# ZwwWayne/mmMOT

Hardware: NVIDIA H100
Metric: frame-pairs/sec at N=128 dets (higher is better)
Workload: dtype f32 (tensor-core engine: FP16 hi/lo split operands, fp32 accumulate)

## Files before the change

mmmot_b200/csrc/gemm_tma.cuh:

```cuda
#pragma once
#include <cuda.h>
#include <cuda_fp16.h>

#include "tc_common.cuh"

namespace tma {

using namespace tc;

constexpr int T_THREADS = 384;
constexpr int T_EPI_WARPS = 8, T_LOAD_WARP = 8;
constexpr int T_CONS_REGS = 232, T_LOAD_REGS = 40;
static_assert(256 * T_CONS_REGS + 128 * T_LOAD_REGS <= launch_regs(T_THREADS) * T_THREADS, "register split exceeds the CTA's pool");
constexpr int T_EPI_SCRATCH = 32 * 80;
constexpr int T_STAGES = 4;
constexpr int T_STAGE_BYTES = A_SUB + 2 * B_HALF;
constexpr size_t T_SMEM_BYTES = (size_t)T_STAGES * T_STAGE_BYTES + 1024 + 256 + T_EPI_WARPS * T_EPI_SCRATCH;
static_assert(T_SMEM_BYTES <= 227 * 1024, "gemm_tma_kernel exceeds the 227 KB of shared memory per block");
static_assert(T_STAGES * T_STAGE_BYTES >= 128 * BN * 4, "the accumulator image must fit in the ring it overlays");

enum { OUT_PLANAR = 3 };

struct TmaP {
  TcP t;
// ... 238 lines not shown
            const uint64_t b_hi = smem_desc_sw64(sb + ks * 32), b_lo = smem_desc_sw64(sb + B_HALF + ks * 32);
#pragma unroll
            for (int mb = 0; mb < 2; mb++) {
              const uint32_t a = sa + mb * 8 * SBO + ks * 2 * A_LBO;
              const uint64_t a_hi = smem_desc(a, A_LBO, SBO), a_lo = smem_desc(a + A_HALF, A_LBO, SBO);
              wgmma_n128(acc[mb], a_hi, b_hi, ((kc - kc_lo) | ks) ? 1u : 0u);
              wgmma_n128(acc[mb], a_hi, b_lo, 1u);
              wgmma_n128(acc[mb], a_lo, b_hi, 1u);
            }
          }
          wgmma_commit();
        }
        wgmma_wait<1>();
        if (kc > kc_lo) { __syncwarp(); if (lane == 0) mbar_arrive(empty_bar((it - 1) % T_STAGES)); }
      }
      wgmma_wait<0>();
      fence_acc(acc[0]);
      fence_acc(acc[1]);
      __syncwarp();
      if (lane == 0) mbar_arrive(empty_bar((it - 1) % T_STAGES));
      bar_sync(7, T_EPI_WARPS * 32);
      acc_dump(acc[0], img, BN, 0, half * 128);
      acc_dump(acc[1], img, BN, 64, half * 128);
      bar_sync(7, T_EPI_WARPS * 32);
      if (P.ksegs > 1) {
        {
          const int co = mg * 128 + q * 32 + lane;
          const bool rowok = co < p.M;
          const float bv = (rowok && p.bias) ? __ldg(p.bias + co) : 0.f;
#pragma unroll 1
          for (int cc = 0; cc < 4; cc++) {
            const int col0 = half * 128 + cc * 32;
            uint32_t v[32];
            acc_ld32(img, BN, q * 32 + lane, col0, v);
            if (!rowok) continue;
            float* sp = P.acc_scratch + ((long)nt * BN + col0) * p.M + co;
            if (seg < P.ksegs - 1) {
              if (seg == 0) {
#pragma unroll
                for (int j = 0; j < 32; j++) __stcg(sp + (long)j * p.M, __uint_as_float(v[j]) * P.t.out_scale);
              } else {
                float sv[32];
#pragma unroll
                for (int j = 0; j < 32; j++) sv[j] = __ldcg(sp + (long)j * p.M);
#pragma unroll
                for (int j = 0; j < 32; j++) __stcg(sp + (long)j * p.M, fmaf(__uint_as_float(v[j]), P.t.out_scale, sv[j]));
              }
            } else {
              float sv[32];
#pragma unroll
              for (int j = 0; j < 32; j++) sv[j] = __ldcg(sp + (long)j * p.M);
#pragma unroll
              for (int j = 0; j < 32; j++) {
                float a = fmaf(__uint_as_float(v[j]), P.t.out_scale, sv[j]) + bv;
                sv[j] = p.relu ? fmaxf(a, 0.f) : a;
              }
              emit_conv(sv, cc, col0, co, i0, y0, x0);
            }
          }
          if (P.pool && seg == P.ksegs - 1 && rowok) pool_flush(co);
        }
      } else
      {
        const int co = mg * 128 + q * 32 + lane;
        const bool rowok = co < p.M;
        const float bv = (rowok && p.bias) ? __ldg(p.bias + co) : 0.f;
        double f1 = 0.0, f2 = 0.0;
        const bool pass2 = P.segsum && !p.part && !p.Y && !p.relu;
        const bool use_seg = p.seg && (p.addend || P.segsum);
        int4 ct = make_int4(0, 0, 0, 0);
        if (use_seg) ct = __ldg(P.chunk_tab + (long)nt * 2 + half);
        const int cdesc[4] = {ct.x, ct.y, ct.z, ct.w};
        float adv[4] = {0.f, 0.f, 0.f, 0.f};
        unsigned one_det = 0;
#pragma unroll
        for (int c = 0; c < 4; c++) {
          if (cdesc[c] & 1) {
            one_det |= 1u << c;
            if (p.addend && rowok) adv[c] = __ldg(p.addend + (long)(cdesc[c] >> 1) * p.ld_add + co);
          }
        }
        float na = 0.f, nb = 0.f;
        if (P.segsum && rowok) { na = __ldg(p.sc + (long)g * p.M + co); nb = __ldg(p.sh + (long)g * p.M + co); }
#pragma unroll 1
        for (int cc = 0; cc < 4; cc++) {
          const int col0 = half * 128 + cc * 32;
          if (col0 >= len) break;
          const int da = (cc == 0 ? ct.x : cc == 1 ? ct.y : cc == 2 ? ct.z : ct.w) >> 1;
          const float adc = cc == 0 ? adv[0] : cc == 1 ? adv[1] : cc == 2 ? adv[2] : adv[3];
          const bool single = (one_det >> cc) & 1u;
          uint32_t v[32];
          acc_ld32(img, BN, q * 32 + lane, col0, v);
          if (P.t.dbg & 1) continue;
          float s1 = 0.f, s2 = 0.f, pv = 0.f;
          bool fast = col0 + 32 <= len;
          if (pass2 && fast) {
            if (single) {
              if (rowok) {
                const float bva = bv + adc;
                const float a2 = P.t.out_scale * na, b2 = fmaf(bva, na, nb);
                float r0 = 0.f, r1 = 0.f;
#pragma unroll
                for (int j = 0; j < 32; j += 2) {
                  r0 += fmaxf(fmaf(__uint_as_float(v[j]), a2, b2), 0.f);
                  r1 += fmaxf(fmaf(__uint_as_float(v[j + 1]), a2, b2), 0.f);
                }
                atomicAdd(P.segsum + (long)da * p.M + co, __float2ull_rn((r0 + r1) * 4294967296.f));
              }
              continue;
            }
          }
          float bva = bv;
          if (fast && p.addend) {
            if (single) bva += adc;
            else fast = false;
          }
          if (fast) {
            if (p.relu) epi_fast<true>(v, P.t.out_scale, bva, pv, s1, s2);
            else epi_fast<false>(v, P.t.out_scale, bva, pv, s1, s2);
          } else {
            float t = 0.f;
#pragma unroll
            for (int j = 0; j < 32; j++) {
              float x = fmaf(__uint_as_float(v[j]), P.t.out_scale, bv);
              const int col = col0 + j;
              if (p.addend && rowok && col < len)
                x += __ldg(p.addend + (long)__ldg(p.seg + c0 + col) * p.ld_add + co);
              if (p.relu) x = fmaxf(x, 0.f);
              v[j] = __float_as_uint(x);
              if (col < len) t += x;
            }
            pv = t / (float)min(32, len - col0);
#pragma unroll
            for (int j = 0; j < 32; j++)
              if (col0 + j < len) { const float d = __uint_as_float(v[j]) - pv; s1 += d; s2 = fmaf(d, d, s2); }
          }
          stat_fold(f1, f2, min(32, len - col0), pv, s1, s2);
          if (P.segsum && rowok) {
            const int nvalid = min(32, len - col0);
            int dcur = da;
            float run = 0.f;
            if (single) {
#pragma unroll
              for (int j = 0; j < 32; j++) run += fmaxf(fmaf(__uint_as_float(v[j]), na, nb), 0.f);
            } else {
#pragma unroll
              for (int j = 0; j < 32; j++) {
                if (j < nvalid) {
                  const int d = __ldg(p.seg + c0 + col0 + j);
                  if (d != dcur) {
                    atomicAdd(P.segsum + (long)dcur * p.M + co, __float2ull_rn(run * 4294967296.f));
                    run = 0.f; dcur = d;
                  }
                  run += fmaxf(fmaf(__uint_as_float(v[j]), na, nb), 0.f);
                }
              }
            }
            atomicAdd(P.segsum + (long)dcur * p.M + co, __float2ull_rn(run * 4294967296.f));
          }
          if (!p.Y || !rowok) continue;
          if (P.conv) {
            float xv[32];
#pragma unroll
            for (int j = 0; j < 32; j++) xv[j] = __uint_as_float(v[j]);
            emit_conv(xv, cc, col0, co, i0, y0, x0);
          } else {
            const int nvalid = min(32, len - col0);
            const long row0 = (long)g * p.y_gs + c0 + col0;
            if (P.t.out_mode == OUT_PLANAR && !(p.y_ms & 31)) {
              float xv[32];
#pragma unroll
              for (int j = 0; j < 32; j++) xv[j] = __uint_as_float(v[j]);
              store_rows(xv, lane < nvalid, (row0 + lane) * p.y_ms + (co - lane));
            } else if (P.t.out_mode == OUT_PLANAR) {
              __half* dst = yh + row0 * p.y_ms + co;
#pragma unroll
              for (int j = 0; j < 32; j++)
                if (j < nvalid) {
                  __half h, l;
                  split_f16(__uint_as_float(v[j]), h, l);
                  amax = fmaxf(amax, fabsf(__uint_as_float(v[j])));
                  dst[(long)j * p.y_ms] = h;
                  dst[(long)j * p.y_ms + P.plane_elems] = l;
                }
            } else {
              float* dst = p.Y + row0 * p.y_ms + co;
              if (nvalid == 32) {
#pragma unroll
                for (int j = 0; j < 32; j++) { *dst = __uint_as_float(v[j]); dst += p.y_ms; }
              } else {
#pragma unroll
                for (int j = 0; j < 32; j++)
                  if (j < nvalid) dst[(long)j * p.y_ms] = __uint_as_float(v[j]);
              }
            }
          }
        }
        if (p.part && rowok) p.part[((long)nt * 2 + half) * p.M + co] = make_double2(f1, f2);
        if (P.conv && P.pool && rowok) pool_flush(co);
      }
      fence_async_smem();
      __syncwarp();
      if (lane == 0) mbar_arrive(free_bar);
      }
    }
    mm_range_flag(P.status, amax);
  } else {
    asm volatile("setmaxnreg.dec.sync.aligned.u32 %0;" ::"n"(T_LOAD_REGS));
    if (warp == T_LOAD_WARP && lane == 0) {
      uint32_t it = 0, wcount = 0;
      for (long t = blockIdx.x; t < total_tiles; t += gridDim.x) {
        const int mg = (int)(t % mgroups);
        const int nt = (int)(t / mgroups);
        const int mt0 = mg;
        int g = 0, c0 = 0, len = BN, i0 = 0, y0 = 0, x0 = 0;
        if (P.conv) conv_origin(nt, i0, y0, x0); else tile_cols(nt, g, c0, len);
        const int row0 = (int)((long)g * p.x_gs + c0);
        for (int kc = 0; kc < KC; kc++, it++) {
          if (kc % P.kc_per_seg == 0) {
            if (wcount > 0) mbar_wait(free_bar, (wcount - 1) & 1);
            wcount++;
          }
          const int s = it % T_STAGES;
          mbar_wait(empty_bar(s), ((it / T_STAGES) & 1) ^ 1);
          const uint32_t abytes = (uint32_t)A_SUB;
          const bool skipA = P.t.dbg & 2, skipB = P.t.dbg & 4;
          mbar_expect_tx(full_bar(s), (skipA ? 0u : abytes) + (skipB ? 0u : 2u * B_HALF));
          const uint32_t sa = base + s * T_STAGE_BYTES, sb = sa + A_SUB;
          const uint8_t* src = reinterpret_cast<const uint8_t*>(P.t.Wp) + ((size_t)kc * P.t.m_tiles + mt0) * A_SUB;
          if (!skipA) bulk_g2s(sa, src, abytes, full_bar(s));
          if (skipB) continue;
          if (P.conv) {
            const int tap = kc / cchunks, cc = kc - tap * cchunks;
            const int dx = tap % 3 - 1, dy = tap / 3 - 1;
            tma_load_4d(sb, &map_hi, cc * BK, x0 + dx, y0 + dy, i0, full_bar(s));
            tma_load_4d(sb + B_HALF, &map_lo, cc * BK, x0 + dx, y0 + dy, i0, full_bar(s));
          } else {
            tma_load_2d(sb, &map_hi, kc * BK, row0, full_bar(s));
            tma_load_2d(sb + B_HALF, &map_lo, kc * BK, row0, full_bar(s));
          }
        }
      }
    }
    __syncwarp();
  }

}

typedef CUresult (*EncodeTiledFn)(CUtensorMap*, CUtensorMapDataType, cuuint32_t, void*, const cuuint64_t*,
                                  const cuuint64_t*, const cuuint32_t*, const cuuint32_t*, CUtensorMapInterleave,
                                  CUtensorMapSwizzle, CUtensorMapL2promotion, CUtensorMapFloatOOBfill);
static inline EncodeTiledFn encode_fn() {
  static EncodeTiledFn fn = nullptr;
  if (!fn) {
    void* p = nullptr;
    cudaDriverEntryPointQueryResult qr;
    if (cudaGetDriverEntryPoint("cuTensorMapEncodeTiled", &p, cudaEnableDefault, &qr) == cudaSuccess &&
        qr == cudaDriverEntryPointSuccess)
      fn = (EncodeTiledFn)p;
  }
  return fn;
}
static inline int make_map_2d(CUtensorMap* m, const void* basep, long rows, int C, long ld) {
  EncodeTiledFn fn = encode_fn();
  if (!fn) return MMMOT_E_ARG;
  cuuint64_t dims[2] = {(cuuint64_t)C, (cuuint64_t)rows};
  cuuint64_t strides[1] = {(cuuint64_t)ld * 2};
  cuuint32_t box[2] = {32, 256}, es[2] = {1, 1};
  CUresult r = fn(m, CU_TENSOR_MAP_DATA_TYPE_FLOAT16, 2, const_cast<void*>(basep), dims, strides, box, es,
                  CU_TENSOR_MAP_INTERLEAVE_NONE, CU_TENSOR_MAP_SWIZZLE_64B, CU_TENSOR_MAP_L2_PROMOTION_L2_128B,
                  CU_TENSOR_MAP_FLOAT_OOB_FILL_NONE);
  return r == CUDA_SUCCESS ? 0 : 900 + (int)r;
}
static inline int make_map_2d_f32(CUtensorMap* m, const void* basep, long rows, int C, int box_rows,
                                  CUtensorMapSwizzle swizzle) {
  EncodeTiledFn fn = encode_fn();
  if (!fn) return MMMOT_E_ARG;
  cuuint64_t dims[2] = {(cuuint64_t)C, (cuuint64_t)rows};
  cuuint64_t strides[1] = {(cuuint64_t)C * 4};
  cuuint32_t box[2] = {32, (cuuint32_t)box_rows}, es[2] = {1, 1};
  CUresult r = fn(m, CU_TENSOR_MAP_DATA_TYPE_FLOAT32, 2, const_cast<void*>(basep), dims, strides, box, es,
                  CU_TENSOR_MAP_INTERLEAVE_NONE, swizzle, CU_TENSOR_MAP_L2_PROMOTION_L2_128B,
                  CU_TENSOR_MAP_FLOAT_OOB_FILL_NONE);
  return r == CUDA_SUCCESS ? 0 : 900 + (int)r;
}
static inline int make_map_4d(CUtensorMap* m, const void* basep, int n_img, int H, int W, int C, int bx, int by,
                              int bi) {
  EncodeTiledFn fn = encode_fn();
  if (!fn) return MMMOT_E_ARG;
  cuuint64_t dims[4] = {(cuuint64_t)C, (cuuint64_t)W, (cuuint64_t)H, (cuuint64_t)n_img};
  cuuint64_t strides[3] = {(cuuint64_t)C * 2, (cuuint64_t)W * C * 2, (cuuint64_t)H * W * C * 2};
  cuuint32_t box[4] = {32, (cuuint32_t)bx, (cuuint32_t)by, (cuuint32_t)bi}, es[4] = {1, 1, 1, 1};
  CUresult r = fn(m, CU_TENSOR_MAP_DATA_TYPE_FLOAT16, 4, const_cast<void*>(basep), dims, strides, box, es,
                  CU_TENSOR_MAP_INTERLEAVE_NONE, CU_TENSOR_MAP_SWIZZLE_64B, CU_TENSOR_MAP_L2_PROMOTION_L2_128B,
                  CU_TENSOR_MAP_FLOAT_OOB_FILL_NONE);
  return r == CUDA_SUCCESS ? 0 : 900 + (int)r;
}

}

#include "gemm_tma_px.cuh"

static int gemm_tma_px_launch(tma::TmaP& P, const CUtensorMap& mh, const CUtensorMap& ml, int sms, cudaStream_t st) {
  static std::atomic<unsigned long long> attr{0};
  MM_TRY(mm_ensure_smem(tma::gemm_tma_px_kernel<false>, tma::PX_SMEM_BYTES, attr));
  const long total = P.t.g.num_tiles;
  const int grid = (int)(total < sms ? total : sms);
  tma::gemm_tma_px_kernel<false><<<grid, tma::PX_THREADS, tma::PX_SMEM_BYTES, st>>>(P, mh, ml);
  MM_LAUNCH_CHECK();
  return 0;
}

static int gemm_tma_px_launch_gen27(const float* crops, int n_img, int H, int W, const uint4* Wpx, float out_scale,
                                    const float* bias, __half* Yhi, long y_plane, int* status, cudaStream_t st) {
  if (!crops || !Wpx || !Yhi) return MMMOT_E_ARG;
  const long n_pix = (long)n_img * H * W;
  if (n_pix >= (1L << 31) || ((long)H * W) % tc::BN || (tc::BN + 2 * W + 2) * 12 > 2 * tma::PX_W_SLOT) return MMMOT_E_SHAPE;
  int sms = 0;
  MM_TRY(mm_sm_count(&sms));
  static std::atomic<unsigned long long> attr{0};
  MM_TRY(mm_ensure_smem(tma::gemm_tma_px_kernel<true>, tma::PX_SMEM_BYTES, attr));
  tma::TmaP P;
  memset(&P, 0, sizeof(P));
  GemmP g = gemm_defaults();
  g.bias = bias; g.M = 64; g.K = 32; g.relu = 1;
  g.S = (int)n_pix; g.tiles_per_group = mm_cdiv(n_pix, tc::BN); g.num_tiles = g.tiles_per_group;
  g.Y = reinterpret_cast<float*>(Yhi); g.y_ms = 64;
  P.t.g = g;
  P.t.Wp = Wpx; P.wcompact = 1;
  P.t.m_tiles = 1; P.t.k_chunks = 1;
  P.t.out_scale = out_scale;
  P.t.out_mode = tma::OUT_PLANAR;
  P.t.dbg = mm_debug_flags();
  P.plane_elems = y_plane;
  P.ksegs = 1; P.kc_per_seg = 1;
  P.status = status;
  P.gen_src = crops; P.n_img = n_img; P.H = H; P.W = W;
  alignas(64) CUtensorMap dummy;
  memset(&dummy, 0, sizeof(dummy));
  const long total = g.num_tiles;
  const int grid = (int)(total < sms ? total : sms);
  tma::gemm_tma_px_kernel<true><<<grid, tma::PX_GEN_THREADS, tma::PX_SMEM_BYTES, st>>>(P, dummy, dummy);
  MM_LAUNCH_CHECK();
  return 0;
}

static int gemm_tma_launch_mat(const GemmP& g, const uint4* Wp, float out_scale, const __half* Xhi, long x_plane,
                               long rows, int ldx, int out_mode, long y_plane, cudaStream_t st,
                               unsigned long long* segsum = nullptr, int* status = nullptr, const int4* chunk_tab = nullptr,
                               const uint4* Wpx = nullptr) {
  if (!Wp || g.num_tiles <= 0 || g.K % tc::BK) return MMMOT_E_ARG;
  int sms = 0;
  MM_TRY(mm_sm_count(&sms));
  static std::atomic<unsigned long long> attr{0};
  MM_TRY(mm_ensure_smem(tma::gemm_tma_kernel, tma::T_SMEM_BYTES, attr));
  tma::TmaP P;
  memset(&P, 0, sizeof(P));
  P.t.g = g;
  P.t.Wp = Wp;
  P.t.m_tiles = (g.M + 127) / 128;
  P.t.k_chunks = g.K / tc::BK;
  P.t.out_scale = out_scale;
  P.t.out_mode = out_mode;
  P.t.dbg = mm_debug_flags();
  P.plane_elems = y_plane;
  P.ksegs = 1; P.kc_per_seg = P.t.k_chunks;
  P.segsum = segsum;
  P.status = status;
  P.chunk_tab = chunk_tab;
  if (g.seg && (g.addend || segsum) && !chunk_tab) return MMMOT_E_ARG;
  alignas(64) CUtensorMap mh, ml;
  MM_TRY(tma::make_map_2d(&mh, Xhi, rows, g.K, ldx));
  MM_TRY(tma::make_map_2d(&ml, Xhi + x_plane, rows, g.K, ldx));
  if (out_mode == tma::OUT_PLANAR && g.M == 64 && g.y_ms == 64 && !g.part && !segsum && !g.addend && !g.tile_tab &&
      !(P.t.dbg & 64)) {
    if (Wpx) { P.t.Wp = Wpx; P.wcompact = 1; }
    return gemm_tma_px_launch(P, mh, ml, sms, st);
  }
  const long total = (long)g.num_tiles * P.t.m_tiles;
  const int grid = (int)(total < sms ? total : sms);
  tma::gemm_tma_kernel<<<grid, tma::T_THREADS, tma::T_SMEM_BYTES, st>>>(P, mh, ml);
  MM_LAUNCH_CHECK();
  return 0;
}

static inline double conv_box_waste(int n_img, int H, int W, int bx, int by, int bi) {
  return (double)mm_cdiv(W, bx) * bx / W * mm_cdiv(H, by) * by / H * mm_cdiv(n_img, bi) * bi / n_img;
}

struct ConvPlan {
  int px;
  int halo;
  int pool;
  int bx, by, bi;
  int ksegs, kc_per_seg;
  int tiles_x, tiles_y, num_tiles;
};
static inline ConvPlan conv_plan(int M, bool part, int n_img, int H, int W, int C, bool want_pool, bool use_kseg, int dbg,
                                 int seg_chunks) {
  ConvPlan c;
  memset(&c, 0, sizeof(c));
  c.bx = 1; c.by = 1; c.bi = 256;
  double best = 1e30;
  for (int cx = 256; cx >= 1; cx >>= 1)
    for (int cy = 256 / cx; cy >= 1; cy >>= 1) {
      const int ci = 256 / (cx * cy);
      const double waste = conv_box_waste(n_img, H, W, cx, cy, ci);
      if (waste < best - 1e-9) { best = waste; c.bx = cx; c.by = cy; c.bi = ci; }
    }
  const int kchunks = 9 * C / tc::BK;
  c.px = M == 64 && !part && !(dbg & 64) && !(use_kseg && seg_chunks > 0 && kchunks > seg_chunks);
  if (c.px && conv_box_waste(1, H, W, 16, 16, 1) <= best + 1e-9) { c.bx = 16; c.by = 16; c.bi = 1; }
  if (c.px) {
    c.halo = (c.bi == 1 && c.bx >= 8 && c.bx * (c.by + 2) * 64 <= tma::PX_X_PLANE && !(dbg & 256)) ? 1 : 0;
    c.pool = want_pool && c.bx >= 2 && c.bx <= 16 && c.by >= 2 && !(H & 1) && !(W & 1) && !(dbg & 512);
  } else {
    c.pool = want_pool && c.bx >= 2 && c.bx <= 32 && c.by >= 2 && !(H & 1) && !(W & 1) && !(dbg & 512);
  }
  c.ksegs = 1; c.kc_per_seg = kchunks;
  if (use_kseg && seg_chunks > 0 && kchunks > seg_chunks) {
    c.ksegs = (kchunks + seg_chunks - 1) / seg_chunks;
    c.kc_per_seg = (kchunks + c.ksegs - 1) / c.ksegs;
  }
  c.tiles_x = mm_cdiv(W, c.bx); c.tiles_y = mm_cdiv(H, c.by);
  c.num_tiles = c.tiles_x * c.tiles_y * mm_cdiv(n_img, c.bi);
  return c;
}

static int gemm_tma_launch_conv(const GemmP& g0, const uint4* Wp, float out_scale, const __half* Xhi, long x_plane,
                                int n_img, int H, int W, int C, __half* Yhi, long y_plane, cudaStream_t st,
                                float* acc_scratch = nullptr, long y_plane_pooled = 0, int* did_pool = nullptr,
                                int* status = nullptr, unsigned long long* pool_sum = nullptr, const uint4* Wpx = nullptr,
                                ConvPlan* plan = nullptr) {
  if (did_pool) *did_pool = 0;
  if (!Wp || C % tc::BK) return MMMOT_E_ARG;
  const ConvPlan c = conv_plan(g0.M, g0.part != nullptr, n_img, H, W, C, y_plane_pooled > 0 && did_pool,
                               acc_scratch != nullptr, mm_debug_flags(), mm_kseg_chunks());
  if (plan) *plan = c;
  int sms = 0;
  MM_TRY(mm_sm_count(&sms));
  static std::atomic<unsigned long long> attr{0};
  MM_TRY(mm_ensure_smem(tma::gemm_tma_kernel, tma::T_SMEM_BYTES, attr));
  tma::TmaP P;
  memset(&P, 0, sizeof(P));
  GemmP g = g0;
  g.K = 9 * C;
  P.conv = 1; P.bx = c.bx; P.by = c.by; P.bi = c.bi;
  P.halo = c.halo;
  P.pool = c.pool;
  if (c.pool) *did_pool = 1;
  if (c.pool && !c.px) P.pool_sum = pool_sum;
  P.tiles_x = c.tiles_x; P.tiles_y = c.tiles_y;
  P.n_img = n_img; P.H = H; P.W = W; P.C = C;
  g.num_tiles = c.num_tiles;
  g.tile_tab = nullptr;
  g.Y = reinterpret_cast<float*>(Yhi);
  g.y_ms = g.M;
  P.t.g = g;
  P.t.Wp = Wp;
  P.t.m_tiles = (g.M + 127) / 128;
  P.t.k_chunks = g.K / tc::BK;
  P.t.out_scale = out_scale;
  P.t.out_mode = tma::OUT_PLANAR;
  P.t.dbg = mm_debug_flags();
  P.plane_elems = P.pool ? y_plane_pooled : y_plane;
  P.status = status;
  P.ksegs = c.ksegs; P.kc_per_seg = c.kc_per_seg;
  if (c.ksegs > 1) P.acc_scratch = acc_scratch;
  alignas(64) CUtensorMap mh, ml;
  const int box_y = P.halo ? c.by + 2 : c.by;
  MM_TRY(tma::make_map_4d(&mh, Xhi, n_img, H, W, C, c.bx, box_y, c.bi));
  MM_TRY(tma::make_map_4d(&ml, Xhi + x_plane, n_img, H, W, C, c.bx, box_y, c.bi));
  if (c.px) {
    if (Wpx) { P.t.Wp = Wpx; P.wcompact = 1; }
    return gemm_tma_px_launch(P, mh, ml, sms, st);
  }
  const long total = (long)g.num_tiles * P.t.m_tiles;
  const int grid = (int)(total < sms ? total : sms);
  tma::gemm_tma_kernel<<<grid, tma::T_THREADS, tma::T_SMEM_BYTES, st>>>(P, mh, ml);
  MM_LAUNCH_CHECK();
  return 0;
}
```

mmmot_b200/csrc/gemm_tma_px.cuh:

```cuda
#pragma once

namespace tma {

constexpr int PX_W_SLOT = 8192;
constexpr int PX_W_LBO = 1024;
constexpr int PX_X_OFF = 3 * PX_W_SLOT;
constexpr int PX_X_PLANE = 24576;
constexpr int PX_STAGE = PX_X_OFF + 2 * PX_X_PLANE;
constexpr int PX_STAGES = 2;
constexpr int PX_IMG = 256 * 64 * 4;
constexpr size_t PX_SMEM_BYTES = (size_t)PX_STAGES * PX_STAGE + PX_IMG + 1024 + 256;

constexpr int PX_WC_LBO = 2048;

constexpr int PX_THREADS = 288, PX_GEN_THREADS = 640, PX_GEN_WARP0 = 12;
constexpr int PX_CONS_REGS = 144, PX_LOAD_REGS = 24, PX_PROD_REGS = 80;
static_assert(256 * PX_CONS_REGS + 128 * PX_LOAD_REGS + 256 * PX_PROD_REGS <= launch_regs(PX_GEN_THREADS) * PX_GEN_THREADS,
              "GEN27 register split exceeds the CTA's pool");

constexpr int PX_GEN_WARPS = 4;

template <bool GEN27>
static __global__ void __launch_bounds__(GEN27 ? PX_GEN_THREADS : PX_THREADS, 1)
gemm_tma_px_kernel(const TmaP P, const __grid_constant__ CUtensorMap map_hi, const __grid_constant__ CUtensorMap map_lo) {
  const GemmP& p = P.t.g;
  extern __shared__ uint8_t smem_raw[];
  __shared__ float s_bias[64];
  const uint32_t raw = smem_u32(smem_raw);
  const uint32_t base = (raw + 1023u) & ~1023u;
  uint8_t* sm = smem_raw + (base - raw);
  float* img = reinterpret_cast<float*>(sm + PX_STAGES * PX_STAGE);
  const uint32_t bar0 = base + PX_STAGES * PX_STAGE + PX_IMG;
  auto full_bar = [&](int s) { return bar0 + 8u * s; };
  auto empty_bar = [&](int s) { return bar0 + 8u * (PX_STAGES + s); };

  const int tid = threadIdx.x, warp = tid >> 5, lane = tid & 31;
  const long total_tiles = p.num_tiles;
  const int KC = P.t.k_chunks;
  const int cchunks = P.conv ? P.C / BK : KC;
  const int ntap = P.halo ? 3 : 1;
  const int nstage = P.halo ? 3 * cchunks : KC;
  const uint32_t xbytes = P.halo ? (uint32_t)(P.bx * (P.by + 2) * 64) : (uint32_t)B_HALF;

  if (tid < 64) s_bias[tid] = p.bias ? p.bias[tid] : 0.f;
  if (tid == 0) {
    for (int s = 0; s < PX_STAGES; s++) {
      mbar_init(full_bar(s), GEN27 ? 1 + PX_GEN_WARPS : 1);
      mbar_init(empty_bar(s), T_EPI_WARPS);
    }
    asm volatile("fence.mbarrier_init.release.cluster;" ::: "memory");
  }
  __syncthreads();

  auto conv_origin = [&](int nt, int& i0, int& y0, int& x0) {
    const int tx = nt % P.tiles_x;
    const int r = nt / P.tiles_x;
    const int ty = r % P.tiles_y;
    i0 = (r / P.tiles_y) * P.bi; y0 = ty * P.by; x0 = tx * P.bx;
  };

  if (warp < T_EPI_WARPS) {
    if (GEN27) asm volatile("setmaxnreg.inc.sync.aligned.u32 %0;" ::"n"(PX_CONS_REGS));
    const int q = warp & 3, cb = (warp >> 2) * 32;
    const int lbx = 31 - __clz(max(P.bx, 1)), lby = 31 - __clz(max(P.by, 1));
    __half* yh = reinterpret_cast<__half*>(p.Y);
    uint32_t racc = 0;
    uint32_t it = 0;
    const int wg = warp >> 2;
    float acc[2][32];
#pragma unroll
    for (int mb = 0; mb < 2; mb++)
#pragma unroll
      for (int i = 0; i < 32; i++) acc[mb][i] = 0.f;
    for (long t = blockIdx.x; t < total_tiles; t += gridDim.x) {
      const int nt = (int)t;
      int i0 = 0, y0 = 0, x0 = 0;
      if (P.conv) conv_origin(nt, i0, y0, x0);
      for (int si = 0; si < nstage; si++, it++) {
        const int s = it % PX_STAGES;
        mbar_wait(full_bar(s), (it / PX_STAGES) & 1);
        const uint32_t sw = base + s * PX_STAGE, sx = sw + PX_X_OFF;
        if (!(P.t.dbg & 8)) {
          wgmma_fence();
          for (int ky = 0; ky < ntap; ky++) {
            const uint32_t xo = sx + (uint32_t)(ky * P.bx * 64 + wg * (128 * 64)), wo = sw + (uint32_t)(ky * PX_W_SLOT);
#pragma unroll
            for (int ks = 0; ks < 2; ks++) {
              uint64_t w_hi, w_lo;
              if (P.wcompact) {
                w_hi = smem_desc(wo + ks * 2 * PX_WC_LBO, PX_WC_LBO, SBO);
                w_lo = smem_desc(wo + 8 * SBO + ks * 2 * PX_WC_LBO, PX_WC_LBO, SBO);
              } else {
                w_hi = smem_desc(wo + ks * 2 * PX_W_LBO, PX_W_LBO, SBO);
                w_lo = smem_desc(wo + PX_W_SLOT / 2 + ks * 2 * PX_W_LBO, PX_W_LBO, SBO);
              }
#pragma unroll
              for (int mb = 0; mb < 2; mb++) {
                const uint64_t x_hi = smem_desc_sw64(xo + mb * (64 * 64) + ks * 32);
                const uint64_t x_lo = smem_desc_sw64(xo + PX_X_PLANE + mb * (64 * 64) + ks * 32);
                wgmma_n64(acc[mb], x_hi, w_hi, (si | ky | ks) ? 1u : 0u);
                wgmma_n64(acc[mb], x_hi, w_lo, 1u);
                wgmma_n64(acc[mb], x_lo, w_hi, 1u);
              }
            }
          }
          wgmma_commit();
        }
        wgmma_wait<1>();
        if (si > 0) { __syncwarp(); if (lane == 0) mbar_arrive(empty_bar((it - 1) % PX_STAGES)); }
      }
      wgmma_wait<0>();
      fence_acc(acc[0]);
      fence_acc(acc[1]);
      __syncwarp();
      if (lane == 0) mbar_arrive(empty_bar((it - 1) % PX_STAGES));
      bar_sync(7, T_EPI_WARPS * 32);
      acc_dump(acc[0], img, 64, wg * 128, 0);
      acc_dump(acc[1], img, 64, wg * 128 + 64, 0);
      bar_sync(7, T_EPI_WARPS * 32);
#pragma unroll 1
      for (int sub = 0; sub < 2; sub++) {
        const int col = sub * 128 + q * 32 + lane;
        bool ok;
        long o;
        if (P.conv) {
          const int xx = col & (P.bx - 1), r = col >> lbx;
          const int yy = r & (P.by - 1), ii = r >> lby;
          const int img = i0 + ii, y = y0 + yy, xg = x0 + xx;
          ok = img < P.n_img && y < P.H && xg < P.W;
          o = (((long)img * P.H + y) * P.W + xg) * 64 + cb;
        } else {
          const long row = (long)nt * BN + col;
          ok = row < p.S;
          o = row * 64 + cb;
        }
        uint32_t v[32];
        acc_ld32(img, 64, sub * 128 + q * 32 + lane, cb, v);
        if (P.t.dbg & 1) continue;
        if (P.pool) {
#pragma unroll
          for (int j = 0; j < 32; j++) {
            float a = __uint_as_float(v[j]);
            a = fmaxf(a, __shfl_xor_sync(0xffffffffu, a, 1));
            a = fmaxf(a, __shfl_xor_sync(0xffffffffu, a, P.bx));
            v[j] = __float_as_uint(a);
          }
          const int xx = col & (P.bx - 1), r = col >> lbx;
          const int yy = r & (P.by - 1);
          const int y = y0 + yy, xg = x0 + xx;
          ok = ok && !(xx & 1) && !(yy & 1);
          o = (((long)(i0 + (r >> lby)) * (P.H >> 1) + (y >> 1)) * (P.W >> 1) + (xg >> 1)) * 64 + cb;
          if (!ok) continue;
        }
        uint32_t hi[16], lo[16];
#pragma unroll
        for (int j = 0; j < 32; j += 2) {
          float x0v = fmaf(__uint_as_float(v[j]), P.t.out_scale, s_bias[cb + j]);
          float x1v = fmaf(__uint_as_float(v[j + 1]), P.t.out_scale, s_bias[cb + j + 1]);
          if (p.relu) { x0v = fmaxf(x0v, 0.f); x1v = fmaxf(x1v, 0.f); }
          split_f16x2(x0v, x1v, hi[j >> 1], lo[j >> 1]);
          mm_range_track2(racc, hi[j >> 1]);
        }
        if (GEN27) {
          const uint32_t scr = base + (uint32_t)((q >> 1) * PX_STAGE + PX_X_OFF + (q & 1) * PX_X_PLANE + 16384);
          const uint32_t rowa = scr + (uint32_t)lane * 128u;
#pragma unroll
          for (int k = 0; k < 4; k++) {
            const uint32_t slot = (uint32_t)((((cb >> 3) + k) ^ (lane & 7)) << 4);
            asm volatile("st.shared.v4.b32 [%0], {%1, %2, %3, %4};" ::"r"(rowa + slot), "r"(hi[4 * k]), "r"(hi[4 * k + 1]),
                         "r"(hi[4 * k + 2]), "r"(hi[4 * k + 3]) : "memory");
            asm volatile("st.shared.v4.b32 [%0], {%1, %2, %3, %4};" ::"r"(rowa + 4096u + slot), "r"(lo[4 * k]),
                         "r"(lo[4 * k + 1]), "r"(lo[4 * k + 2]), "r"(lo[4 * k + 3]) : "memory");
          }
          asm volatile("bar.sync %0, 64;" ::"r"(3 + q) : "memory");
          const int h = warp >> 2;
          const long row0 = (long)nt * BN + sub * 128 + q * 32;
          __half* dstp = yh + (long)h * P.plane_elems + row0 * 64;
#pragma unroll
          for (int r = 0; r < 4; r++) {
            const int idx = r * 32 + lane, px = idx >> 2, c = (idx & 3) * 2;
            const uint32_t ra = scr + (uint32_t)h * 4096u + (uint32_t)px * 128u;
            uint32_t w[8];
            asm volatile("ld.shared.v4.b32 {%0, %1, %2, %3}, [%4];" : "=r"(w[0]), "=r"(w[1]), "=r"(w[2]), "=r"(w[3])
                         : "r"(ra + (uint32_t)((c ^ (px & 7)) << 4)));
            asm volatile("ld.shared.v4.b32 {%0, %1, %2, %3}, [%4];" : "=r"(w[4]), "=r"(w[5]), "=r"(w[6]), "=r"(w[7])
                         : "r"(ra + (uint32_t)(((c + 1) ^ (px & 7)) << 4)));
            if (row0 + px < p.S) st_global_256(dstp + (long)px * 64 + c * 8, w);
          }
          asm volatile("bar.sync %0, 64;" ::"r"(3 + q) : "memory");
        } else if (ok && !(P.t.dbg & 128)) {
          st_global_256(yh + o, hi);
          st_global_256(yh + o + 16, hi + 8);
          st_global_256(yh + o + P.plane_elems, lo);
          st_global_256(yh + o + P.plane_elems + 16, lo + 8);
        } else if (ok) {
          uint4* dh = reinterpret_cast<uint4*>(yh + o);
          uint4* dl = reinterpret_cast<uint4*>(yh + o + P.plane_elems);
#pragma unroll
          for (int k = 0; k < 4; k++) {
            dh[k] = make_uint4(hi[4 * k], hi[4 * k + 1], hi[4 * k + 2], hi[4 * k + 3]);
            dl[k] = make_uint4(lo[4 * k], lo[4 * k + 1], lo[4 * k + 2], lo[4 * k + 3]);
          }
        }
      }
    }
    mm_range_flag2(P.status, racc);
  } else if (GEN27 && warp >= PX_GEN_WARP0) {
    asm volatile("setmaxnreg.dec.sync.aligned.u32 %0;" ::"n"(PX_PROD_REGS));
    const int pw = warp - PX_GEN_WARP0;
    const int grp = pw >> 2;
    const int pt = (pw & 3) * 32 + lane;
    const int W = P.W, hw = P.H * P.W;
    const int span = BN + 2 * W + 2;
    float amax = 0.f;
    uint32_t it = (uint32_t)grp;
    for (long t = blockIdx.x + (long)grp * gridDim.x; t < total_tiles; t += 2L * gridDim.x, it += 2) {
      const int s = it % PX_STAGES;
      const long row0 = t * BN;
      const long img = row0 / hw;
      const int r0 = (int)(row0 - img * hw);
      const float* src = P.gen_src + img * 3 * hw;
      mbar_wait(empty_bar(s), ((it / PX_STAGES) & 1) ^ 1);
      float* stg = reinterpret_cast<float*>(sm + s * PX_STAGE + PX_W_SLOT);
      const int lin0 = r0 - W - 1;
      if (P.t.dbg & 4) {
        __syncwarp();
        if (lane == 0) mbar_arrive(full_bar(s));
        continue;
      }
#pragma unroll 1
      for (int i0 = pt; i0 < 3 * span; i0 += 8 * 128) {
        float q[8];
#pragma unroll
        for (int u = 0; u < 8; u++) {
          const int i = i0 + u * 128;
          const int ci = i / span, lin = lin0 + (i - ci * span);
          q[u] = (i < 3 * span && lin >= 0 && lin < hw) ? __ldg(src + (long)ci * hw + lin) : 0.f;
        }
#pragma unroll
        for (int u = 0; u < 8; u++)
          if (i0 + u * 128 < 3 * span) stg[i0 + u * 128] = q[u];
      }
      asm volatile("bar.sync %0, 128;" ::"r"(1 + grp) : "memory");
      const uint32_t sx = base + s * PX_STAGE + PX_X_OFF;
#pragma unroll
      for (int j = 0; j < 2; j++) {
        const int rr = j * 128 + pt;
        const int x = (r0 + rr) % W;
        const bool xl = x > 0, xr = x < W - 1;
        const float* c = stg + rr + W + 1;
        float v[28];
#pragma unroll
        for (int ci = 0; ci < 3; ci++)
#pragma unroll
          for (int ky = 0; ky < 3; ky++)
#pragma unroll
            for (int kx = 0; kx < 3; kx++) {
              float q = c[ci * span + (ky - 1) * W + (kx - 1)];
              if (kx == 0 && !xl) q = 0.f;
              if (kx == 2 && !xr) q = 0.f;
              v[ci * 9 + ky * 3 + kx] = q;
              amax = fmaxf(amax, fabsf(q));
            }
        v[27] = 0.f;
        uint32_t hi[16], lo[16];
#pragma unroll
        for (int k = 0; k < 28; k += 2) split_f16x2(v[k], v[k + 1], hi[k >> 1], lo[k >> 1]);
        hi[14] = hi[15] = lo[14] = lo[15] = 0u;
        const uint32_t rowaddr = sx + (uint32_t)rr * 64u, sw = (uint32_t)((rr >> 1) & 3);
#pragma unroll
        for (int cch = 0; cch < 4; cch++) {
          const uint32_t a = rowaddr + ((cch ^ sw) << 4);
          asm volatile("st.shared.v4.b32 [%0], {%1, %2, %3, %4};" ::"r"(a), "r"(hi[4 * cch]), "r"(hi[4 * cch + 1]),
                       "r"(hi[4 * cch + 2]), "r"(hi[4 * cch + 3]) : "memory");
          asm volatile("st.shared.v4.b32 [%0], {%1, %2, %3, %4};" ::"r"(a + PX_X_PLANE), "r"(lo[4 * cch]),
                       "r"(lo[4 * cch + 1]), "r"(lo[4 * cch + 2]), "r"(lo[4 * cch + 3]) : "memory");
        }
      }
      asm volatile("fence.proxy.async.shared::cta;" ::: "memory");
      __syncwarp();
      if (lane == 0) mbar_arrive(full_bar(s));
    }
    mm_range_flag(P.status, amax);
  } else {
    if (GEN27) asm volatile("setmaxnreg.dec.sync.aligned.u32 %0;" ::"n"(PX_LOAD_REGS));
    if (warp == T_LOAD_WARP && lane == 0) {
      uint32_t it = 0;
      for (long t = blockIdx.x; t < total_tiles; t += gridDim.x) {
        const int nt = (int)t;
        int i0 = 0, y0 = 0, x0 = 0;
        if (P.conv) conv_origin(nt, i0, y0, x0);
        for (int si = 0; si < nstage; si++, it++) {
          const int s = it % PX_STAGES;
          mbar_wait(empty_bar(s), ((it / PX_STAGES) & 1) ^ 1);
          mbar_expect_tx(full_bar(s), (uint32_t)ntap * PX_W_SLOT + (GEN27 ? 0u : 2u * xbytes));
          const uint32_t sw = base + s * PX_STAGE, sx = sw + PX_X_OFF;
          const int kx = P.halo ? si / cchunks : 0, cc = P.halo ? si - kx * cchunks : 0;
          for (int ky = 0; ky < ntap; ky++) {
            const int kc = P.halo ? (ky * 3 + kx) * cchunks + cc : si;
            if (P.wcompact) {
              bulk_g2s(sw + ky * PX_W_SLOT, reinterpret_cast<const uint8_t*>(P.t.Wp) + (size_t)kc * PX_W_SLOT, PX_W_SLOT, full_bar(s));
            } else {
              const uint8_t* src = reinterpret_cast<const uint8_t*>(P.t.Wp) + (size_t)kc * P.t.m_tiles * A_SUB;
#pragma unroll
              for (int r = 0; r < 8; r++)
                bulk_g2s(sw + ky * PX_W_SLOT + r * PX_W_LBO, src + r * A_LBO, 1024, full_bar(s));
            }
          }
          if (P.halo) {
            tma_load_4d(sx, &map_hi, cc * BK, x0 + kx - 1, y0 - 1, i0, full_bar(s));
            tma_load_4d(sx + PX_X_PLANE, &map_lo, cc * BK, x0 + kx - 1, y0 - 1, i0, full_bar(s));
          } else if (P.conv) {
            const int tap = si / cchunks, c2 = si - tap * cchunks;
            const int dx = tap % 3 - 1, dy = tap / 3 - 1;
            tma_load_4d(sx, &map_hi, c2 * BK, x0 + dx, y0 + dy, i0, full_bar(s));
            tma_load_4d(sx + PX_X_PLANE, &map_lo, c2 * BK, x0 + dx, y0 + dy, i0, full_bar(s));
          } else if (!GEN27) {
            tma_load_2d(sx, &map_hi, si * BK, nt * BN, full_bar(s));
            tma_load_2d(sx + PX_X_PLANE, &map_lo, si * BK, nt * BN, full_bar(s));
          }
        }
      }
    }
    __syncwarp();
  }
}

}
```

Before: 195.9.

## Offload px-kernel epilogue to dedicated warps and template the tap count

In the non-GEN27 px GEMM kernel, the consumer warps now only dump accumulators into the shared image and signal an mbarrier. Four new epilogue warps do the scale, bias, split and store work, so the next tile's wgmma can overlap the previous tile's epilogue. The tap count becomes a template parameter (1 or 3) so the tap loop unrolls and weight descriptors are computed without a branch. Debug flags can now skip W or X loads. The single shared accumulator image serialises dump and epilogue through the img_full/img_free barriers. More threads per CTA reduce the register budget per thread.

```diff
diff --git a/mmmot_b200/csrc/gemm_tma.cuh b/mmmot_b200/csrc/gemm_tma.cuh
--- a/mmmot_b200/csrc/gemm_tma.cuh
+++ b/mmmot_b200/csrc/gemm_tma.cuh
@@ -564,11 +564,16 @@
 #include "gemm_tma_px.cuh"
 
 static int gemm_tma_px_launch(tma::TmaP& P, const CUtensorMap& mh, const CUtensorMap& ml, int sms, cudaStream_t st) {
-  static std::atomic<unsigned long long> attr{0};
-  MM_TRY(mm_ensure_smem(tma::gemm_tma_px_kernel<false>, tma::PX_SMEM_BYTES, attr));
+  static std::atomic<unsigned long long> attr_halo{0}, attr_tap{0};
   const long total = P.t.g.num_tiles;
   const int grid = (int)(total < sms ? total : sms);
-  tma::gemm_tma_px_kernel<false><<<grid, tma::PX_THREADS, tma::PX_SMEM_BYTES, st>>>(P, mh, ml);
+  if (P.halo) {
+    MM_TRY(mm_ensure_smem(tma::gemm_tma_px_kernel<false, 3>, tma::PX_SMEM_BYTES, attr_halo));
+    tma::gemm_tma_px_kernel<false, 3><<<grid, tma::PX_THREADS, tma::PX_SMEM_BYTES, st>>>(P, mh, ml);
+  } else {
+    MM_TRY(mm_ensure_smem(tma::gemm_tma_px_kernel<false, 1>, tma::PX_SMEM_BYTES, attr_tap));
+    tma::gemm_tma_px_kernel<false, 1><<<grid, tma::PX_THREADS, tma::PX_SMEM_BYTES, st>>>(P, mh, ml);
+  }
   MM_LAUNCH_CHECK();
   return 0;
 }
@@ -581,7 +586,7 @@
   int sms = 0;
   MM_TRY(mm_sm_count(&sms));
   static std::atomic<unsigned long long> attr{0};
-  MM_TRY(mm_ensure_smem(tma::gemm_tma_px_kernel<true>, tma::PX_SMEM_BYTES, attr));
+  MM_TRY(mm_ensure_smem(tma::gemm_tma_px_kernel<true, 1>, tma::PX_SMEM_BYTES, attr));
   tma::TmaP P;
   memset(&P, 0, sizeof(P));
   GemmP g = gemm_defaults();
@@ -602,7 +607,7 @@
   memset(&dummy, 0, sizeof(dummy));
   const long total = g.num_tiles;
   const int grid = (int)(total < sms ? total : sms);
-  tma::gemm_tma_px_kernel<true><<<grid, tma::PX_GEN_THREADS, tma::PX_SMEM_BYTES, st>>>(P, dummy, dummy);
+  tma::gemm_tma_px_kernel<true, 1><<<grid, tma::PX_GEN_THREADS, tma::PX_SMEM_BYTES, st>>>(P, dummy, dummy);
   MM_LAUNCH_CHECK();
   return 0;
 }
diff --git a/mmmot_b200/csrc/gemm_tma_px.cuh b/mmmot_b200/csrc/gemm_tma_px.cuh
--- a/mmmot_b200/csrc/gemm_tma_px.cuh
+++ b/mmmot_b200/csrc/gemm_tma_px.cuh
@@ -13,16 +13,19 @@
 
 constexpr int PX_WC_LBO = 2048;
 
-constexpr int PX_THREADS = 288, PX_GEN_THREADS = 640, PX_GEN_WARP0 = 12;
+constexpr int PX_THREADS = 416, PX_EPI_WARP0 = 9, PX_EPI_WARPS = 4;
+constexpr int PX_GEN_THREADS = 640, PX_GEN_WARP0 = 12;
 constexpr int PX_CONS_REGS = 144, PX_LOAD_REGS = 24, PX_PROD_REGS = 80;
 static_assert(256 * PX_CONS_REGS + 128 * PX_LOAD_REGS + 256 * PX_PROD_REGS <= launch_regs(PX_GEN_THREADS) * PX_GEN_THREADS,
               "GEN27 register split exceeds the CTA's pool");
 
 constexpr int PX_GEN_WARPS = 4;
 
-template <bool GEN27>
+template <bool GEN27, int NTAP>
 static __global__ void __launch_bounds__(GEN27 ? PX_GEN_THREADS : PX_THREADS, 1)
 gemm_tma_px_kernel(const TmaP P, const __grid_constant__ CUtensorMap map_hi, const __grid_constant__ CUtensorMap map_lo) {
+  static_assert(NTAP == 1 || (NTAP == 3 && !GEN27), "a stage serves 1 tap, or 3 from a halo box");
+  constexpr bool HALO = NTAP == 3;
   const GemmP& p = P.t.g;
   extern __shared__ uint8_t smem_raw[];
   __shared__ float s_bias[64];
@@ -33,14 +36,14 @@
   const uint32_t bar0 = base + PX_STAGES * PX_STAGE + PX_IMG;
   auto full_bar = [&](int s) { return bar0 + 8u * s; };
   auto empty_bar = [&](int s) { return bar0 + 8u * (PX_STAGES + s); };
+  const uint32_t img_full = bar0 + 8u * (2 * PX_STAGES), img_free = img_full + 8u;
 
   const int tid = threadIdx.x, warp = tid >> 5, lane = tid & 31;
   const long total_tiles = p.num_tiles;
   const int KC = P.t.k_chunks;
   const int cchunks = P.conv ? P.C / BK : KC;
-  const int ntap = P.halo ? 3 : 1;
-  const int nstage = P.halo ? 3 * cchunks : KC;
-  const uint32_t xbytes = P.halo ? (uint32_t)(P.bx * (P.by + 2) * 64) : (uint32_t)B_HALF;
+  const int nstage = HALO ? 3 * cchunks : KC;
+  const uint32_t xbytes = HALO ? (uint32_t)(P.bx * (P.by + 2) * 64) : (uint32_t)B_HALF;
 
   if (tid < 64) s_bias[tid] = p.bias ? p.bias[tid] : 0.f;
   if (tid == 0) {
@@ -48,6 +51,8 @@
       mbar_init(full_bar(s), GEN27 ? 1 + PX_GEN_WARPS : 1);
       mbar_init(empty_bar(s), T_EPI_WARPS);
     }
+    mbar_init(img_full, T_EPI_WARPS * 32);
+    mbar_init(img_free, PX_EPI_WARPS * 32);
     asm volatile("fence.mbarrier_init.release.cluster;" ::: "memory");
   }
   __syncthreads();
@@ -59,20 +64,107 @@
     i0 = (r / P.tiles_y) * P.bi; y0 = ty * P.by; x0 = tx * P.bx;
   };
 
+  const int lbx = 31 - __clz(max(P.bx, 1)), lby = 31 - __clz(max(P.by, 1));
+  __half* yh = reinterpret_cast<__half*>(p.Y);
+  auto epilogue = [&](int nt, int i0, int y0, int x0, int sub, int q, int cb, uint32_t& racc) {
+    const int col = sub * 128 + q * 32 + lane;
+    bool ok;
+    long o;
+    if (P.conv) {
+      const int xx = col & (P.bx - 1), r = col >> lbx;
+      const int yy = r & (P.by - 1), ii = r >> lby;
+      const int img = i0 + ii, y = y0 + yy, xg = x0 + xx;
+      ok = img < P.n_img && y < P.H && xg < P.W;
+      o = (((long)img * P.H + y) * P.W + xg) * 64 + cb;
+    } else {
+      const long row = (long)nt * BN + col;
+      ok = row < p.S;
+      o = row * 64 + cb;
+    }
+    uint32_t v[32];
+    acc_ld32(img, 64, sub * 128 + q * 32 + lane, cb, v);
+    if (P.t.dbg & 1) return;
+    if (P.pool) {
+#pragma unroll
+      for (int j = 0; j < 32; j++) {
+        float a = __uint_as_float(v[j]);
+        a = fmaxf(a, __shfl_xor_sync(0xffffffffu, a, 1));
+        a = fmaxf(a, __shfl_xor_sync(0xffffffffu, a, P.bx));
+        v[j] = __float_as_uint(a);
+      }
+      const int xx = col & (P.bx - 1), r = col >> lbx;
+      const int yy = r & (P.by - 1);
+      const int y = y0 + yy, xg = x0 + xx;
+      ok = ok && !(xx & 1) && !(yy & 1);
+      o = (((long)(i0 + (r >> lby)) * (P.H >> 1) + (y >> 1)) * (P.W >> 1) + (xg >> 1)) * 64 + cb;
+      if (!ok) return;
+    }
+    uint32_t hi[16], lo[16];
+#pragma unroll
+    for (int j = 0; j < 32; j += 2) {
+      float x0v = fmaf(__uint_as_float(v[j]), P.t.out_scale, s_bias[cb + j]);
+      float x1v = fmaf(__uint_as_float(v[j + 1]), P.t.out_scale, s_bias[cb + j + 1]);
+      if (p.relu) { x0v = fmaxf(x0v, 0.f); x1v = fmaxf(x1v, 0.f); }
+      split_f16x2(x0v, x1v, hi[j >> 1], lo[j >> 1]);
+      mm_range_track2(racc, hi[j >> 1]);
+    }
+    if (GEN27) {
+      const uint32_t scr = base + (uint32_t)((q >> 1) * PX_STAGE + PX_X_OFF + (q & 1) * PX_X_PLANE + 16384);
+      const uint32_t rowa = scr + (uint32_t)lane * 128u;
+#pragma unroll
+      for (int k = 0; k < 4; k++) {
+        const uint32_t slot = (uint32_t)((((cb >> 3) + k) ^ (lane & 7)) << 4);
+        asm volatile("st.shared.v4.b32 [%0], {%1, %2, %3, %4};" ::"r"(rowa + slot), "r"(hi[4 * k]), "r"(hi[4 * k + 1]),
+                     "r"(hi[4 * k + 2]), "r"(hi[4 * k + 3]) : "memory");
+        asm volatile("st.shared.v4.b32 [%0], {%1, %2, %3, %4};" ::"r"(rowa + 4096u + slot), "r"(lo[4 * k]),
+                     "r"(lo[4 * k + 1]), "r"(lo[4 * k + 2]), "r"(lo[4 * k + 3]) : "memory");
+      }
+      asm volatile("bar.sync %0, 64;" ::"r"(3 + q) : "memory");
+      const int h = warp >> 2;
+      const long row0 = (long)nt * BN + sub * 128 + q * 32;
+      __half* dstp = yh + (long)h * P.plane_elems + row0 * 64;
+#pragma unroll
+      for (int r = 0; r < 4; r++) {
+        const int idx = r * 32 + lane, px = idx >> 2, c = (idx & 3) * 2;
+        const uint32_t ra = scr + (uint32_t)h * 4096u + (uint32_t)px * 128u;
+        uint32_t w[8];
+        asm volatile("ld.shared.v4.b32 {%0, %1, %2, %3}, [%4];" : "=r"(w[0]), "=r"(w[1]), "=r"(w[2]), "=r"(w[3])
+                     : "r"(ra + (uint32_t)((c ^ (px & 7)) << 4)));
+        asm volatile("ld.shared.v4.b32 {%0, %1, %2, %3}, [%4];" : "=r"(w[4]), "=r"(w[5]), "=r"(w[6]), "=r"(w[7])
+                     : "r"(ra + (uint32_t)(((c + 1) ^ (px & 7)) << 4)));
+        if (row0 + px < p.S) st_global_256(dstp + (long)px * 64 + c * 8, w);
+      }
+      asm volatile("bar.sync %0, 64;" ::"r"(3 + q) : "memory");
+    } else if (ok && !(P.t.dbg & 128)) {
+      st_global_256(yh + o, hi);
+      st_global_256(yh + o + 16, hi + 8);
+      st_global_256(yh + o + P.plane_elems, lo);
+      st_global_256(yh + o + P.plane_elems + 16, lo + 8);
+    } else if (ok) {
+      uint4* dh = reinterpret_cast<uint4*>(yh + o);
+      uint4* dl = reinterpret_cast<uint4*>(yh + o + P.plane_elems);
+#pragma unroll
+      for (int k = 0; k < 4; k++) {
+        dh[k] = make_uint4(hi[4 * k], hi[4 * k + 1], hi[4 * k + 2], hi[4 * k + 3]);
+        dl[k] = make_uint4(lo[4 * k], lo[4 * k + 1], lo[4 * k + 2], lo[4 * k + 3]);
+      }
+    }
+  };
+
   if (warp < T_EPI_WARPS) {
     if (GEN27) asm volatile("setmaxnreg.inc.sync.aligned.u32 %0;" ::"n"(PX_CONS_REGS));
-    const int q = warp & 3, cb = (warp >> 2) * 32;
-    const int lbx = 31 - __clz(max(P.bx, 1)), lby = 31 - __clz(max(P.by, 1));
-    __half* yh = reinterpret_cast<__half*>(p.Y);
     uint32_t racc = 0;
     uint32_t it = 0;
+    uint32_t n = 0;
     const int wg = warp >> 2;
+    const uint32_t w_lbo = P.wcompact ? PX_WC_LBO : PX_W_LBO;
+    const uint32_t w_lo_off = P.wcompact ? 8 * SBO : PX_W_SLOT / 2;
     float acc[2][32];
 #pragma unroll
     for (int mb = 0; mb < 2; mb++)
 #pragma unroll
       for (int i = 0; i < 32; i++) acc[mb][i] = 0.f;
-    for (long t = blockIdx.x; t < total_tiles; t += gridDim.x) {
+    for (long t = blockIdx.x; t < total_tiles; t += gridDim.x, n++) {
       const int nt = (int)t;
       int i0 = 0, y0 = 0, x0 = 0;
       if (P.conv) conv_origin(nt, i0, y0, x0);
@@ -82,18 +174,13 @@
         const uint32_t sw = base + s * PX_STAGE, sx = sw + PX_X_OFF;
         if (!(P.t.dbg & 8)) {
           wgmma_fence();
-          for (int ky = 0; ky < ntap; ky++) {
+#pragma unroll
+          for (int ky = 0; ky < NTAP; ky++) {
             const uint32_t xo = sx + (uint32_t)(ky * P.bx * 64 + wg * (128 * 64)), wo = sw + (uint32_t)(ky * PX_W_SLOT);
 #pragma unroll
             for (int ks = 0; ks < 2; ks++) {
-              uint64_t w_hi, w_lo;
-              if (P.wcompact) {
-                w_hi = smem_desc(wo + ks * 2 * PX_WC_LBO, PX_WC_LBO, SBO);
-                w_lo = smem_desc(wo + 8 * SBO + ks * 2 * PX_WC_LBO, PX_WC_LBO, SBO);
-              } else {
-                w_hi = smem_desc(wo + ks * 2 * PX_W_LBO, PX_W_LBO, SBO);
-                w_lo = smem_desc(wo + PX_W_SLOT / 2 + ks * 2 * PX_W_LBO, PX_W_LBO, SBO);
-              }
+              const uint64_t w_hi = smem_desc(wo + ks * 2 * w_lbo, w_lbo, SBO);
+              const uint64_t w_lo = smem_desc(wo + w_lo_off + ks * 2 * w_lbo, w_lbo, SBO);
 #pragma unroll
               for (int mb = 0; mb < 2; mb++) {
                 const uint64_t x_hi = smem_desc_sw64(xo + mb * (64 * 64) + ks * 32);
@@ -114,95 +201,34 @@
       fence_acc(acc[1]);
       __syncwarp();
       if (lane == 0) mbar_arrive(empty_bar((it - 1) % PX_STAGES));
-      bar_sync(7, T_EPI_WARPS * 32);
-      acc_dump(acc[0], img, 64, wg * 128, 0);
-      acc_dump(acc[1], img, 64, wg * 128 + 64, 0);
-      bar_sync(7, T_EPI_WARPS * 32);
+      if constexpr (GEN27) {
+        bar_sync(7, T_EPI_WARPS * 32);
+        acc_dump(acc[0], img, 64, wg * 128, 0);
+        acc_dump(acc[1], img, 64, wg * 128 + 64, 0);
+        bar_sync(7, T_EPI_WARPS * 32);
 #pragma unroll 1
-      for (int sub = 0; sub < 2; sub++) {
-        const int col = sub * 128 + q * 32 + lane;
-        bool ok;
-        long o;
-        if (P.conv) {
-          const int xx = col & (P.bx - 1), r = col >> lbx;
-          const int yy = r & (P.by - 1), ii = r >> lby;
-          const int img = i0 + ii, y = y0 + yy, xg = x0 + xx;
-          ok = img < P.n_img && y < P.H && xg < P.W;
-          o = (((long)img * P.H + y) * P.W + xg) * 64 + cb;
-        } else {
-          const long row = (long)nt * BN + col;
-          ok = row < p.S;
-          o = row * 64 + cb;
-        }
-        uint32_t v[32];
-        acc_ld32(img, 64, sub * 128 + q * 32 + lane, cb, v);
-        if (P.t.dbg & 1) continue;
-        if (P.pool) {
-#pragma unroll
-          for (int j = 0; j < 32; j++) {
-            float a = __uint_as_float(v[j]);
-            a = fmaxf(a, __shfl_xor_sync(0xffffffffu, a, 1));
-            a = fmaxf(a, __shfl_xor_sync(0xffffffffu, a, P.bx));
-            v[j] = __float_as_uint(a);
-          }
-          const int xx = col & (P.bx - 1), r = col >> lbx;
-          const int yy = r & (P.by - 1);
-          const int y = y0 + yy, xg = x0 + xx;
-          ok = ok && !(xx & 1) && !(yy & 1);
-          o = (((long)(i0 + (r >> lby)) * (P.H >> 1) + (y >> 1)) * (P.W >> 1) + (xg >> 1)) * 64 + cb;
-          if (!ok) continue;
-        }
-        uint32_t hi[16], lo[16];
-#pragma unroll
-        for (int j = 0; j < 32; j += 2) {
-          float x0v = fmaf(__uint_as_float(v[j]), P.t.out_scale, s_bias[cb + j]);
-          float x1v = fmaf(__uint_as_float(v[j + 1]), P.t.out_scale, s_bias[cb + j + 1]);
-          if (p.relu) { x0v = fmaxf(x0v, 0.f); x1v = fmaxf(x1v, 0.f); }
-          split_f16x2(x0v, x1v, hi[j >> 1], lo[j >> 1]);
-          mm_range_track2(racc, hi[j >> 1]);
-        }
-        if (GEN27) {
-          const uint32_t scr = base + (uint32_t)((q >> 1) * PX_STAGE + PX_X_OFF + (q & 1) * PX_X_PLANE + 16384);
-          const uint32_t rowa = scr + (uint32_t)lane * 128u;
-#pragma unroll
-          for (int k = 0; k < 4; k++) {
-            const uint32_t slot = (uint32_t)((((cb >> 3) + k) ^ (lane & 7)) << 4);
-            asm volatile("st.shared.v4.b32 [%0], {%1, %2, %3, %4};" ::"r"(rowa + slot), "r"(hi[4 * k]), "r"(hi[4 * k + 1]),
-                         "r"(hi[4 * k + 2]), "r"(hi[4 * k + 3]) : "memory");
-            asm volatile("st.shared.v4.b32 [%0], {%1, %2, %3, %4};" ::"r"(rowa + 4096u + slot), "r"(lo[4 * k]),
-                         "r"(lo[4 * k + 1]), "r"(lo[4 * k + 2]), "r"(lo[4 * k + 3]) : "memory");
-          }
-          asm volatile("bar.sync %0, 64;" ::"r"(3 + q) : "memory");
-          const int h = warp >> 2;
-          const long row0 = (long)nt * BN + sub * 128 + q * 32;
-          __half* dstp = yh + (long)h * P.plane_elems + row0 * 64;
-#pragma unroll
-          for (int r = 0; r < 4; r++) {
-            const int idx = r * 32 + lane, px = idx >> 2, c = (idx & 3) * 2;
-            const uint32_t ra = scr + (uint32_t)h * 4096u + (uint32_t)px * 128u;
-            uint32_t w[8];
-            asm volatile("ld.shared.v4.b32 {%0, %1, %2, %3}, [%4];" : "=r"(w[0]), "=r"(w[1]), "=r"(w[2]), "=r"(w[3])
-                         : "r"(ra + (uint32_t)((c ^ (px & 7)) << 4)));
-            asm volatile("ld.shared.v4.b32 {%0, %1, %2, %3}, [%4];" : "=r"(w[4]), "=r"(w[5]), "=r"(w[6]), "=r"(w[7])
-                         : "r"(ra + (uint32_t)(((c + 1) ^ (px & 7)) << 4)));
-            if (row0 + px < p.S) st_global_256(dstp + (long)px * 64 + c * 8, w);
-          }
-          asm volatile("bar.sync %0, 64;" ::"r"(3 + q) : "memory");
-        } else if (ok && !(P.t.dbg & 128)) {
-          st_global_256(yh + o, hi);
-          st_global_256(yh + o + 16, hi + 8);
-          st_global_256(yh + o + P.plane_elems, lo);
-          st_global_256(yh + o + P.plane_elems + 16, lo + 8);
-        } else if (ok) {
-          uint4* dh = reinterpret_cast<uint4*>(yh + o);
-          uint4* dl = reinterpret_cast<uint4*>(yh + o + P.plane_elems);
-#pragma unroll
-          for (int k = 0; k < 4; k++) {
-            dh[k] = make_uint4(hi[4 * k], hi[4 * k + 1], hi[4 * k + 2], hi[4 * k + 3]);
-            dl[k] = make_uint4(lo[4 * k], lo[4 * k + 1], lo[4 * k + 2], lo[4 * k + 3]);
-          }
-        }
-      }
+        for (int sub = 0; sub < 2; sub++) epilogue(nt, i0, y0, x0, sub, warp & 3, (warp >> 2) * 32, racc);
+      } else {
+        mbar_wait(img_free, (n & 1) ^ 1);
+        acc_dump(acc[0], img, 64, wg * 128, 0);
+        acc_dump(acc[1], img, 64, wg * 128 + 64, 0);
+        mbar_arrive(img_full);
+      }
+    }
+    if (GEN27) mm_range_flag2(P.status, racc);
+  } else if (!GEN27 && warp >= PX_EPI_WARP0) {
+    const int q = warp - PX_EPI_WARP0;
+    uint32_t racc = 0, n = 0;
+    for (long t = blockIdx.x; t < total_tiles; t += gridDim.x, n++) {
+      const int nt = (int)t;
+      int i0 = 0, y0 = 0, x0 = 0;
+      if (P.conv) conv_origin(nt, i0, y0, x0);
+      mbar_wait(img_full, n & 1);
+#pragma unroll 1
+      for (int cb = 0; cb < 64; cb += 32)
+#pragma unroll 1
+        for (int sub = 0; sub < 2; sub++) epilogue(nt, i0, y0, x0, sub, q, cb, racc);
+      mbar_arrive(img_free);
     }
     mm_range_flag2(P.status, racc);
   } else if (GEN27 && warp >= PX_GEN_WARP0) {
@@ -293,11 +319,12 @@
         for (int si = 0; si < nstage; si++, it++) {
           const int s = it % PX_STAGES;
           mbar_wait(empty_bar(s), ((it / PX_STAGES) & 1) ^ 1);
-          mbar_expect_tx(full_bar(s), (uint32_t)ntap * PX_W_SLOT + (GEN27 ? 0u : 2u * xbytes));
+          const bool skipW = P.t.dbg & 2, skipX = GEN27 || (P.t.dbg & 4);
+          mbar_expect_tx(full_bar(s), (skipW ? 0u : (uint32_t)NTAP * PX_W_SLOT) + (skipX ? 0u : 2u * xbytes));
           const uint32_t sw = base + s * PX_STAGE, sx = sw + PX_X_OFF;
-          const int kx = P.halo ? si / cchunks : 0, cc = P.halo ? si - kx * cchunks : 0;
-          for (int ky = 0; ky < ntap; ky++) {
-            const int kc = P.halo ? (ky * 3 + kx) * cchunks + cc : si;
+          const int kx = HALO ? si / cchunks : 0, cc = HALO ? si - kx * cchunks : 0;
+          for (int ky = 0; ky < NTAP && !skipW; ky++) {
+            const int kc = HALO ? (ky * 3 + kx) * cchunks + cc : si;
             if (P.wcompact) {
               bulk_g2s(sw + ky * PX_W_SLOT, reinterpret_cast<const uint8_t*>(P.t.Wp) + (size_t)kc * PX_W_SLOT, PX_W_SLOT, full_bar(s));
             } else {
@@ -307,7 +334,8 @@
                 bulk_g2s(sw + ky * PX_W_SLOT + r * PX_W_LBO, src + r * A_LBO, 1024, full_bar(s));
             }
           }
-          if (P.halo) {
+          if (skipX) continue;
+          if (HALO) {
             tma_load_4d(sx, &map_hi, cc * BK, x0 + kx - 1, y0 - 1, i0, full_bar(s));
             tma_load_4d(sx + PX_X_PLANE, &map_lo, cc * BK, x0 + kx - 1, y0 - 1, i0, full_bar(s));
           } else if (P.conv) {
@@ -315,7 +343,7 @@
             const int dx = tap % 3 - 1, dy = tap / 3 - 1;
             tma_load_4d(sx, &map_hi, c2 * BK, x0 + dx, y0 + dy, i0, full_bar(s));
             tma_load_4d(sx + PX_X_PLANE, &map_lo, c2 * BK, x0 + dx, y0 + dy, i0, full_bar(s));
-          } else if (!GEN27) {
+          } else {
             tma_load_2d(sx, &map_hi, si * BK, nt * BN, full_bar(s));
             tma_load_2d(sx + PX_X_PLANE, &map_lo, si * BK, nt * BN, full_bar(s));
           }
```

After: 201.2 (median of 6 runs). +2.7%, better.
